# Lucaskabela/UNAST

Measured on AMD Instinct MI355X. Metric: mel-frames/sec/node (train step, gen+disc) at B=32,T_mel=800; 1/2/4/8-GPU scaling, higher is better.
Workload: dtype bf16x3

## Files before the change

### include/unast_hip.h

```cpp
#ifndef UNAST_HIP_H
#define UNAST_HIP_H
#include <stdint.h>
#ifdef __cplusplus
extern "C" {
#endif

typedef struct ihipStream_t* hipStream_t;

const char* unast_last_error(void);
int unast_version(void);
const char* unast_arch(void);

int unast_gemm(int a_mode, int b_mode, int nsplit,
               const float* A, int lda, const float* B, int ldb, float* C, int ldc,
               int M, int N, int K, int kb_valid,
               int conv_T, int conv_ca, int conv_cb, int conv_shift,
               const float* bias, const float* R, int ldr, const float* G, int ldg, float gate_scale,
               float alpha, int beta, int act,
               float drop_p, unsigned int seed, unsigned int stream_id,
               int splitk, float* splitk_ws, int64_t splitk_ws_floats, float* rowsum_a, int tile_wn, int b_presplit,
               int out_split, double* colstats, hipStream_t stream);

int unast_attn_fwd(int nsplit, const float* Q, int ldq, const float* K, int ldk, const float* V, int ldv, float* O, int ldo,
                   float* LSE, const int* lens_k, int B, int H, int Tq, int Tk, int head_dim, int causal, float scale,
// ... 83 lines not shown
                        double* ws, float* loss, hipStream_t stream);
int unast_text_loss_bwd(const float* logits, int ldl, const int64_t* gold, int rows, int V, float eos_weight, const double* ws,
                        const float* gscale, float* dlogits, hipStream_t stream);
int unast_text_head_loss(const float* X, int ldx, const float* W, const float* bias, const int64_t* gold, int rows, int K, int V,
                         float eos_weight, float gscale, float* logits, float* dlogits, int ldl, double* ws, float* loss, hipStream_t stream);
int unast_speech_head_loss(const float* X, int ldx, const float* W, const float* bias, const float* gold, const int* lens, int B, int T, int K, int M,
                           float eos_weight, float gscale, float* head, float* d_head, int ldh, double* ws, hipStream_t stream);
int unast_speech_post_loss(const float* gold, const float* post, const int* lens, int B, int T, int M, float gscale, float* d_post, double* ws,
                           float* loss, hipStream_t stream);
int unast_disc_targets(const int64_t* perm, int n, int B, int flip, float smoothing, float* out, hipStream_t stream);
int unast_randperm(int64_t* out, int n, unsigned int seed, unsigned int stream_id, hipStream_t stream);
int unast_bce_logits(const float* logits, int ldx, const float* targets, int n, const float* gscale, float* loss, float* dlogits,
                     int ldd, hipStream_t stream);

int unast_lstm_fwd(const float* xproj, const float* whh, const float* b_ih, const float* b_hh, const int* lens, float* y, float* gates,
                   float* cs, float* hprev, float* hfinal, int Bd, int T, int ndir, int hidden, int64_t whh_dir_stride,
                   int64_t bias_dir_stride, hipStream_t stream);
int unast_lstm_bwd(const float* dy, const float* dhfinal, const float* whh, const float* gates, const float* cs, const int* lens,
                   float* dgates, int Bd, int T, int ndir, int hidden, int64_t whh_dir_stride, hipStream_t stream);
int unast_leaky_dropout(const float* x, const float* dy, float* out, int rows, int D, float slope, float drop_p, unsigned int seed,
                        unsigned int stream_id, hipStream_t stream);

int unast_conv_fwd(int nsplit, const float* X, int ldx, const float* Wp, float* Y, int ldy, int B, int T, int Cin, int Cout,
                   int taps, int pad_left, const float* bias, int act, const float* R, int ldr, hipStream_t stream);
int unast_maxpool_prev(const float* in, int ld_in, float* out, int ld_out, int B, int T, int C, hipStream_t stream);
int unast_highway_combine(const float* ht, int ld_ht, const float* x, int ld_x, float* out, int ld_out, int rows, int C, hipStream_t stream);
int unast_gru_fwd(const float* xproj, const float* whh, const float* b_hn, float* y, int B, int T, int hidden, hipStream_t stream);

int unast_set_rng_epoch(const unsigned int* counter);

typedef struct {
    const float* A; int lda;
    const float* B; int ldb;
    float* C; int ldc;
    float* rowsum_a;
    int M, N, K;
} unast_wgrad_item;
int unast_wgrad_group(int nsplit, int count, const unast_wgrad_item* items, float* ws, int64_t ws_floats, int target_blocks,
                      hipStream_t stream);
int64_t unast_wgrad_group_ws_floats(int count, const unast_wgrad_item* items, int target_blocks);

int unast_sumsq(const float* g, int64_t n, double* out, hipStream_t stream);
int unast_adamw(float* p, float* g, float* m, float* v, int64_t n, const double* sumsq, float max_norm, float lr,
                float beta1, float beta2, float eps, float weight_decay, int step, float* split_out, int decoupled,
                const float* dev_hyper, int zero_grad, hipStream_t stream);
int unast_split_f32(const float* src, float* dst, int64_t n, hipStream_t stream);
int unast_transpose_split(const float* src_base, float* dst_base, const int* tiles_dev, int ntiles, hipStream_t stream);

int unast_panel_gemm(const float* A, int lda, const void* w_planes, int64_t plane_bytes, float* C, int ldc, int M, int N, int K,
                     const float* bias, const float* R, int ldr, const float* G, int ldg, float gate_scale, int act,
                     float drop_p, unsigned int seed, unsigned int stream_id, int out_split,
                     const float* ln_gamma, const float* ln_beta, float* Y, int ldy, float* mean, float* rstd, float eps,
                     void* gate_bits, int rows_per_wg, hipStream_t stream);
int unast_retile_weights(const float* src_base, void* dst_base, const void* descs_dev, int ndesc, hipStream_t stream);
int unast_panel_gemm_lnbwd(const float* A, int lda, const void* w_planes, int64_t plane_bytes, int M, int K, const float* R, int ldr,
                           const float* z, int ldz, const float* mean, const float* rstd, const float* gamma,
                           float* dz, int lddz, float* dz_drop, int lddrop, float* part, int64_t part_floats,
                           float drop_p, unsigned int seed, unsigned int stream_id, hipStream_t stream);
int64_t unast_panel_gemm_lnbwd_ws_floats(int M);
int unast_layernorm_partials_finalize(const float* part, int nblk, int C, float* dgamma, float* dbeta, hipStream_t stream);
int unast_set_words(unsigned int* dst, const unsigned int* host_words, int n, hipStream_t stream);

int64_t unast_graph_plan_create(void* graph, int nstreams);
int unast_graph_plan_info(int64_t plan, int* out4);
int unast_graph_plan_replay(int64_t plan, hipStream_t origin);
int unast_graph_plan_destroy(int64_t plan);
int unast_graph_plan_allreduces(int64_t plan);
int unast_graph_plan_set_comm(int64_t plan, int64_t comm);
int unast_graph_plan_allreduce_counts(int64_t plan, long long* out, int n);
int unast_capture_reset(void);
int unast_capture_note(hipStream_t stream);
int unast_capture_get_deps(hipStream_t stream, void** out, int cap);
int unast_capture_prune(hipStream_t stream, hipStream_t origin, void** keep, int nkeep);
int unast_graph_plan_streams(int64_t plan);

int unast_comm_unique_id(void* out128);
int64_t unast_comm_init(const void* unique_id128, int rank, int world);
int unast_allreduce(int64_t comm, float* buf, int64_t count, hipStream_t stream);
int unast_allreduce_marker(float* buf, int64_t count, hipStream_t stream);
int unast_comm_destroy(int64_t comm);

#ifdef __cplusplus
}
#endif
#endif
```

### unast_amd/config.py

```python
import os

NSPLIT = 1 if os.environ.get("UNAST_PREC", "bf16x3").lower() in ("bf16", "1") else 3


def set_precision(name):
    global NSPLIT
    NSPLIT = {"bf16": 1, "bf16x3": 3}[name]


def precision_name():
    return "bf16" if NSPLIT == 1 else "bf16x3"


def snapshot():
    return tuple(sorted((k, v) for k, v in globals().items() if k.isupper()))


SIDE_STREAMS = os.environ.get("UNAST_SIDE_STREAMS", "1") != "0"

DECODE_GRAPH = os.environ.get("UNAST_DECODE_GRAPH", "1") != "0"

WGRAD_STREAM_MIN_TOKENS = int(os.environ.get("UNAST_WGRAD_MIN_TOKENS", "8192"))

DETERMINISTIC_SUMS = os.environ.get("UNAST_DETERMINISTIC_SUMS", "0") == "1"

CAPTURE_PRUNE = os.environ.get("UNAST_CAPTURE_PRUNE", "1") != "0"

WGRAD_GROUP = os.environ.get("UNAST_WGRAD_GROUP", "1") != "0"

ATTN_FUSED_BWD = os.environ.get("UNAST_ATTN_FUSED_BWD", "1") != "0"
ATTN_BWD_TERMS = int(os.environ.get("UNAST_ATTN_BWD_TERMS", "3"))

DGRAD_TRANSPOSED = os.environ.get("UNAST_DGRAD_T", "0") == "1"

PANEL_MIN_ROWS = int(os.environ.get("UNAST_PANEL_MIN_ROWS", "16384"))
PANEL_ROWS = int(os.environ.get("UNAST_PANEL_ROWS", "1128"))

NATIVE_COMM = os.environ.get("UNAST_NATIVE_COMM", "1") != "0"

ENC_SKIP_PAD_GRADS = os.environ.get("UNAST_ENC_SKIP_PAD_GRADS", "0") == "1"

STREAM_JITTER = int(os.environ.get("UNAST_STREAM_JITTER", "0"))
STREAM_JITTER_SEED = int(os.environ.get("UNAST_STREAM_JITTER_SEED", "0"))

DEBUG_WORKSPACES = os.environ.get("UNAST_DEBUG_WORKSPACES", "0") == "1"

JOINT_GEN = os.environ.get("UNAST_JOINT_GEN", "1") != "0"
```

### unast_amd/csrc/panel.hip

```cpp
#include "common.h"
#include <algorithm>
#include "../../include/unast_hip.h"
#include <type_traits>

static unsigned long long* g_panel_stamps = nullptr;
#define PSUB 1024

struct PanelParams {
    const float* A; int lda;
    const unsigned char* W; size_t plane_bytes;
    float* C; int ldc;
    int M, N, K, ncg;
    const float* bias; const float* R; int ldr;
    const float* G; int ldg; float gate_scale;
    int act; uint32_t drop_thresh; float drop_scale; uint32_t seed, stream;
    int out_split;
    const float* gamma; const float* beta; float* Y; int ldy; float* mean; float* rstd; float eps;
    const float* Z; int ldz; float* part;
    unsigned long long* gate_bits;
    unsigned long long* stamps;
};

__device__ __forceinline__ void panel_wait_vm(int n) {
#define PW(k) asm volatile("s_waitcnt vmcnt(" #k ")" ::: "memory")
    if (n < 8) {
        if (n < 4) { if (n < 2) PW(0); else PW(2); }
        else       { if (n < 6) PW(4); else PW(6); }
    } else if (n < 16) {
        if (n < 12) { if (n < 10) PW(8); else PW(10); }
        else        { if (n < 14) PW(12); else PW(14); }
    } else {
        if (n < 20) PW(16); else PW(20);
    }
#undef PW
}

#ifdef PANEL_STAMPS
__device__ __forceinline__ unsigned long long panel_stamp() {
    unsigned long long t;
    asm volatile("s_memtime %0\n\ts_waitcnt lgkmcnt(0)" : "=s"(t) :: "memory");
    return t;
}
#define STAMP(var) const unsigned long long var = panel_stamp()
#define STAMP_ADD(slot, a, b) stamp_sum[slot] += (b) - (a)
#else
#define STAMP(var)
#define STAMP_ADD(slot, a, b)
#endif

template <int KSTEPS, int RT, int LN, int NW>
__global__ __launch_bounds__(64 * NW, NW / 4) void panel_kernel(const PanelParams p) {
    constexpr int NT = 64 * NW, ROWS = (NW / 2) * 16 * RT;
    constexpr int NSUB = 8 * KSTEPS;
    constexpr int GROUP = NSUB * PSUB;
    constexpr int DMAX = (NSUB + NW - 1) / NW;
    constexpr int RING = 2 * GROUP;
    constexpr bool A_DMA = (KSTEPS == 8);
    static_assert(!A_DMA || RING >= ROWS * 1024, "the A image borrows the ring");
    __shared__ __attribute__((aligned(16))) unsigned char smem[(RING > ROWS * 1024 || !A_DMA ? RING : ROWS * 1024) + 4096 + 1024];

    const int t = threadIdx.x, lane = t & 63, l15 = lane & 15, g = lane >> 4;
    const int wave = __builtin_amdgcn_readfirstlane(t >> 6);
    __builtin_assume(wave >= 0 && wave < NW);
    const int rg = wave >> 1, ch = wave & 1;
    const int m_wg = blockIdx.x * ROWS;
    const int m_wave = m_wg + rg * (16 * RT);
#ifdef PANEL_STAMPS
    unsigned long long stamp_sum[8] = {0, 0, 0, 0, 0, 0, 0, 0};
    const unsigned long long t_begin = panel_stamp();
#endif
    const uint32_t rbase = p.drop_thresh ? rng_stream_base(p.seed, p.stream) : 0u;

    const __amdgpu_buffer_rsrc_t w_rsrc = __builtin_amdgcn_make_buffer_rsrc(const_cast<unsigned char*>(p.W), 0, 0x7FFFFFF0, 0x00020000);
    const int lane16 = lane * 16;
    auto issue_group = [&](int cg) {
#pragma unroll
        for (int q = 0; q < DMAX; ++q) {
            const int j = wave + NW * q;
            if (j >= NSUB) break;
            const int pl = j / (4 * KSTEPS), rem = j - pl * (4 * KSTEPS);
            const uint32_t soff = (uint32_t)pl * (uint32_t)p.plane_bytes + (uint32_t)(4 * cg * KSTEPS + rem) * PSUB;
            __builtin_amdgcn_raw_ptr_buffer_load_lds(w_rsrc, (__attribute__((address_space(3))) void*)(smem + (cg & 1) * GROUP + j * PSUB), 16, lane16, (int)soff, 0, 0);
        }
    };

    float* const sbias = reinterpret_cast<float*>(smem + RING);
    float* const sred = sbias + 1024;
    const uint32_t sbias_lds = (uint32_t)(uintptr_t)(__attribute__((address_space(3))) void*)sbias;
    const bool bias_lds = p.bias && p.N <= 1024;
    if (bias_lds) {
        for (int i = t; i < 64 * p.ncg; i += NT) sbias[i] = (i < p.N) ? p.bias[i] : 0.f;
    }

    bf16x8_t ah[RT][KSTEPS], al[RT][KSTEPS];
    if constexpr (A_DMA) {
        const __amdgpu_buffer_rsrc_t a_rsrc = __builtin_amdgcn_make_buffer_rsrc(const_cast<float*>(p.A), 0, 0x7FFFFFF0, 0x00020000);
#pragma unroll
        for (int q = 0; q < ROWS / NW; ++q) {
            const int r = wave * (ROWS / NW) + q;
            const int row = min(m_wg + r, p.M - 1);
            __builtin_amdgcn_raw_ptr_buffer_load_lds(a_rsrc, (__attribute__((address_space(3))) void*)(smem + r * 1024), 16, (lane ^ (r & 15)) << 4,
                                                     (int)((uint32_t)row * (uint32_t)p.lda * 4u), 0, 0);
        }
        asm volatile("s_waitcnt vmcnt(0)" ::: "memory");
        __syncthreads();
#pragma unroll
        for (int rt = 0; rt < RT; ++rt) {
            const unsigned char* rowp = smem + (rg * (16 * RT) + 16 * rt + l15) * 1024;
#pragma unroll
            for (int ks = 0; ks < KSTEPS; ++ks) {
                const int c0 = 8 * ks + 2 * g;
                const float4 a = *reinterpret_cast<const float4*>(rowp + ((c0 ^ l15) << 4));
                const float4 c = *reinterpret_cast<const float4*>(rowp + (((c0 + 1) ^ l15) << 4));
                u32x2 h0, l0, h1, l1;
                split4<3>(a, h0, l0);
                split4<3>(c, h1, l1);
                ah[rt][ks] = __builtin_bit_cast(bf16x8_t, (u32x4){h0[0], h0[1], h1[0], h1[1]});
                al[rt][ks] = __builtin_bit_cast(bf16x8_t, (u32x4){l0[0], l0[1], l1[0], l1[1]});
            }
        }
        __syncthreads();
    } else {
#pragma unroll
        for (int rt = 0; rt < RT; ++rt) {
            const int row = min(m_wave + 16 * rt + l15, p.M - 1);
            const float* ar = p.A + (size_t)row * p.lda;
#pragma unroll
            for (int ks = 0; ks < KSTEPS; ++ks) {
                const int k = 32 * ks + 8 * g;
                const int k0 = min(k, p.K - 4), k1 = min(k + 4, p.K - 4);
                float4 a = *reinterpret_cast<const float4*>(ar + k0);
                float4 c = *reinterpret_cast<const float4*>(ar + k1);
                if (k >= p.K) a = make_float4(0.f, 0.f, 0.f, 0.f);
                if (k + 4 >= p.K) c = make_float4(0.f, 0.f, 0.f, 0.f);
                u32x2 h0, l0, h1, l1;
                split4<3>(a, h0, l0);
                split4<3>(c, h1, l1);
                ah[rt][ks] = __builtin_bit_cast(bf16x8_t, (u32x4){h0[0], h0[1], h1[0], h1[1]});
                al[rt][ks] = __builtin_bit_cast(bf16x8_t, (u32x4){l0[0], l0[1], l1[0], l1[1]});
            }
        }
        __syncthreads();
    }
    issue_group(0);
#ifdef PANEL_STAMPS
    { const unsigned long long tp = panel_stamp(); stamp_sum[5] = tp - t_begin; }
#endif

    const bool vec_c = (p.ldc & 3) == 0;
    const bool vec_r = p.R && (p.ldr & 3) == 0 && ((((uintptr_t)p.R) & 15) == 0);
    const bool vec_g = p.G && (p.ldg & 3) == 0 && ((((uintptr_t)p.G) & 15) == 0);
    const int lane_off = (g * 16 + l15) * 16;

    auto epilogue = [&](int cg, f32x4 (&ac)[RT][2]) {
#pragma unroll
        for (int rt = 0; rt < RT; ++rt) {
            const int m = m_wave + 16 * rt + l15;
            if (m >= p.M) continue;
            uint32_t rkey = 0;
            if (p.drop_thresh) rkey = pcg_hash((uint32_t)m + rbase);
#pragma unroll
            for (int c2 = 0; c2 < 2; ++c2) {
                const int n = 64 * cg + 32 * ch + 16 * c2 + 4 * g;
                if (n >= p.N) continue;
                float v[4] = {ac[rt][c2][0], ac[rt][c2][1], ac[rt][c2][2], ac[rt][c2][3]};
                float bv[4] = {0.f, 0.f, 0.f, 0.f}, gv[4] = {1.f, 1.f, 1.f, 1.f}, rv[4] = {0.f, 0.f, 0.f, 0.f};
                const bool full = n + 3 < p.N;
                if (p.bias) {
#pragma unroll
                    for (int r = 0; r < 4; ++r) bv[r] = (n + r < p.N) ? p.bias[n + r] : 0.f;
                }
                if (p.G) {
                    if (full && vec_g) { const float4 t4 = *reinterpret_cast<const float4*>(p.G + (size_t)m * p.ldg + n); gv[0] = t4.x; gv[1] = t4.y; gv[2] = t4.z; gv[3] = t4.w; }
                    else { for (int r = 0; r < 4; ++r) if (n + r < p.N) gv[r] = p.G[(size_t)m * p.ldg + n + r]; }
                }
                if (p.R) {
                    if (full && vec_r) { const float4 t4 = *reinterpret_cast<const float4*>(p.R + (size_t)m * p.ldr + n); rv[0] = t4.x; rv[1] = t4.y; rv[2] = t4.z; rv[3] = t4.w; }
                    else { for (int r = 0; r < 4; ++r) if (n + r < p.N) rv[r] = p.R[(size_t)m * p.ldr + n + r]; }
                }
#pragma unroll
                for (int r = 0; r < 4; ++r) {
                    float x = v[r] + bv[r];
                    if (p.act == 1) x = fmaxf(x, 0.f);
                    if (p.drop_thresh) x = rng_keep(rkey, (uint32_t)(n + r), p.drop_thresh) ? x * p.drop_scale : 0.f;
                    if (p.G) x = (gv[r] > 0.f) ? x * p.gate_scale : 0.f;
                    v[r] = x + rv[r];
                }
                float* cp = p.C + (size_t)m * p.ldc + n;
                if (full && vec_c) {
                    const float4 o = make_float4(v[0], v[1], v[2], v[3]);
                    if (p.out_split) *reinterpret_cast<uint4*>(cp) = split_chunk(o);
                    else *reinterpret_cast<float4*>(cp) = o;
                } else {
                    for (int r = 0; r < 4; ++r) if (n + r < p.N) cp[r] = v[r];
                }
            }
        }
    };
    const __amdgpu_buffer_rsrc_t c_rsrc = __builtin_amdgcn_make_buffer_rsrc(p.C, 0, (int)min((size_t)0x7FFFFFF0, ((size_t)(p.M - 1) * p.ldc + p.N) * 4), 0x00020000);
    uint32_t c_voff[RT], c_rkey[RT];
#pragma unroll
    for (int rt = 0; rt < RT; ++rt) {
        const int m = m_wave + 16 * rt + l15;
        c_voff[rt] = ((uint32_t)m * (uint32_t)p.ldc + (uint32_t)(32 * ch + 4 * g)) * 4u;
        c_rkey[rt] = pcg_hash((uint32_t)m + rbase);
    }
    const int ntile_n = (p.N + 15) >> 4, ntile_m = (p.M + 15) >> 4;
    const __amdgpu_buffer_rsrc_t g_rsrc = __builtin_amdgcn_make_buffer_rsrc(p.gate_bits, 0, ((p.M + 127) >> 7) * 8 * ntile_n * 32, 0x00020000);
    auto epilogue_fast = [&](int cg, f32x4 (&ac)[RT][2], auto act_t, auto drop_t, auto split_t, auto wbits_t, auto rgate_t) {
        constexpr bool ACT = decltype(act_t)::value, DROP = decltype(drop_t)::value, SPLIT = decltype(split_t)::value;
        constexpr bool WBITS = decltype(wbits_t)::value, RGATE = decltype(rgate_t)::value;
        f32x4 b4[2] = {(f32x4){0.f, 0.f, 0.f, 0.f}, (f32x4){0.f, 0.f, 0.f, 0.f}};
        if (bias_lds) {
            const uint32_t ba = sbias_lds + 4u * (uint32_t)(64 * cg + 32 * ch + 4 * g);
            asm volatile("ds_read_b128 %0, %2\n\tds_read_b128 %1, %2 offset:64\n\ts_waitcnt lgkmcnt(0)" : "=&v"(b4[0]), "=&v"(b4[1]) : "v"(ba) : "memory");
        }
        const int soff = cg * 256;
#pragma unroll
        for (int rt = 0; rt < RT; ++rt) {
#pragma unroll
            for (int c2 = 0; c2 < 2; ++c2) {
                float v[4] = {ac[rt][c2][0] + b4[c2][0], ac[rt][c2][1] + b4[c2][1], ac[rt][c2][2] + b4[c2][2], ac[rt][c2][3] + b4[c2][3]};
                if (ACT) {
#pragma unroll
                    for (int r = 0; r < 4; ++r) asm("v_max_f32 %0, 0, %1" : "=v"(v[r]) : "v"(v[r]));
                }
                if (DROP) {
                    const uint32_t n = (uint32_t)(64 * cg + 32 * ch + 16 * c2 + 4 * g);
                    const uint32_t h01 = rng_pair(c_rkey[rt], n), h23 = rng_pair(c_rkey[rt], n + 2u);
                    v[0] = rng_keep_lo(h01, p.drop_thresh) ? v[0] * p.drop_scale : 0.f;
                    v[1] = rng_keep_hi(h01, p.drop_thresh) ? v[1] * p.drop_scale : 0.f;
                    v[2] = rng_keep_lo(h23, p.drop_thresh) ? v[2] * p.drop_scale : 0.f;
                    v[3] = rng_keep_hi(h23, p.drop_thresh) ? v[3] * p.drop_scale : 0.f;
                }
                if (WBITS || RGATE) {
                    const int tile_m = RGATE ? min((m_wave >> 4) + rt, ntile_m - 1) : (m_wave >> 4) + rt;
                    const int widx = ((tile_m * ntile_n) + 4 * cg + 2 * ch + c2) * 4;
                    if (WBITS) {
                        const unsigned long long b0 = __ballot(v[0] > 0.f), b1 = __ballot(v[1] > 0.f), b2 = __ballot(v[2] > 0.f), b3 = __ballot(v[3] > 0.f);
                        const unsigned long long mine = lane == 0 ? b0 : lane == 1 ? b1 : lane == 2 ? b2 : b3;
                        if (lane < 4) __builtin_amdgcn_raw_buffer_store_b64((u32x2){(uint32_t)mine, (uint32_t)(mine >> 32)}, g_rsrc, (widx + lane) * 8, 0, 0);
                    } else {
                        const __attribute__((address_space(4))) unsigned long long* wp = (const __attribute__((address_space(4))) unsigned long long*)(uintptr_t)p.gate_bits + widx;
#pragma unroll
                        for (int r = 0; r < 4; ++r) v[r] = ((wp[r] >> lane) & 1ull) ? v[r] * p.gate_scale : 0.f;
                    }
                }
                u32x4 o;
                if (SPLIT) {
                    const uint4 sc = split_chunk(make_float4(v[0], v[1], v[2], v[3]));
                    o = (u32x4){sc.x, sc.y, sc.z, sc.w};
                } else {
                    o = (u32x4){__float_as_uint(v[0]), __float_as_uint(v[1]), __float_as_uint(v[2]), __float_as_uint(v[3])};
                }
                __builtin_amdgcn_raw_buffer_store_b128(o, c_rsrc, (int)(c_voff[rt] + (uint32_t)soff) + 64 * c2, 0, 0);
            }
        }
    };
    const int s_fast = 2 * RT;
    int st_prev = 0, st_now = 0;
    const bool fast_ok = vec_c && !p.R && !p.G && (bias_lds || !p.bias);
    const int epi_kind = !fast_ok ? 0 : p.gate_bits ? (p.act == 1 ? (p.out_split ? 0 : p.drop_thresh ? 5 : 7) : (!p.drop_thresh && !p.out_split && !p.bias ? 6 : 0))
                       : p.drop_thresh ? (p.act == 1 && !p.out_split ? 1 : 0) : p.out_split ? (p.act == 1 ? 0 : 2) : (p.act == 1 ? 3 : 4);
    const int s_epi = s_fast + (epi_kind == 5 || epi_kind == 7 ? 2 * RT : 0);
    auto run_epilogue = [&](int cg, f32x4 (&ac)[RT][2]) {
        STAMP(te0);
        using T = std::true_type; using F = std::false_type;
#ifdef PKO_PLAIN_EPILOGUE
        if (64 * cg + 64 <= p.N) { epilogue_fast(cg, ac, F{}, F{}, F{}, F{}, F{}); st_now += s_fast; return; }
#endif
#ifdef PKO_NO_EPILOGUE
        if (64 * cg + 64 <= p.N) { asm volatile("" :: "v"(ac[0][0]), "v"(ac[0][1])); return; }
#endif
        if (epi_kind == 0 || 64 * cg + 64 > p.N) {
            epilogue(cg, ac);
        } else {
            __builtin_amdgcn_s_setprio(1);
            if (epi_kind == 1) epilogue_fast(cg, ac, T{}, T{}, F{}, F{}, F{});
            else if (epi_kind == 2) epilogue_fast(cg, ac, F{}, F{}, T{}, F{}, F{});
            else if (epi_kind == 3) epilogue_fast(cg, ac, T{}, F{}, F{}, F{}, F{});
            else if (epi_kind == 5) epilogue_fast(cg, ac, T{}, T{}, F{}, T{}, F{});
            else if (epi_kind == 6) epilogue_fast(cg, ac, F{}, F{}, F{}, F{}, T{});
            else if (epi_kind == 7) epilogue_fast(cg, ac, T{}, F{}, F{}, T{}, F{});
            else epilogue_fast(cg, ac, F{}, F{}, F{}, F{}, F{});
            __builtin_amdgcn_s_setprio(0);
            st_now += s_epi;
        }
        STAMP(te1);
        STAMP_ADD(3, te0, te1);
    };

    auto group_sync = [&](int cg) {
        STAMP(ta);
        panel_wait_vm(st_prev);
        STAMP(tb);
        __builtin_amdgcn_s_barrier();
        STAMP(tc);
        if (cg + 1 < p.ncg) issue_group(cg + 1);
        STAMP(td);
        STAMP_ADD(0, ta, tb); STAMP_ADD(1, tb, tc); STAMP_ADD(2, tc, td);
    };
    auto group_mma = [&](int cg, auto k0_t, auto k1_t, f32x4 (&ac)[RT][2]) {
        constexpr int K0 = decltype(k0_t)::value, K1 = decltype(k1_t)::value;
        if constexpr (K0 < K1) {
            const unsigned char* base = smem + (cg & 1) * GROUP + lane_off + (2 * ch) * KSTEPS * PSUB;
            bf16x8_t bf[2][2][2];
            auto load_b = [&](int buf, int ks) {
#pragma unroll
                for (int c2 = 0; c2 < 2; ++c2) {
                    bf[buf][c2][0] = *reinterpret_cast<const bf16x8_t*>(base + ((0 * 4 + c2) * KSTEPS + ks) * PSUB);
                    bf[buf][c2][1] = *reinterpret_cast<const bf16x8_t*>(base + ((1 * 4 + c2) * KSTEPS + ks) * PSUB);
                }
            };
            STAMP(tm0);
            load_b(K0 & 1, K0);
#ifdef PKO_NO_LDS_READS
            load_b((K0 + 1) & 1, K0);
#endif
#pragma unroll
            for (int ks = K0; ks < K1; ++ks) {
#ifndef PKO_NO_LDS_READS
                if (ks + 1 < K1) load_b((ks + 1) & 1, ks + 1);
#endif
#pragma unroll
                for (int c2 = 0; c2 < 2; ++c2) {
                    const bf16x8_t bh = bf[ks & 1][c2][0], bl = bf[ks & 1][c2][1];
#pragma unroll
                    for (int rt = 0; rt < RT; ++rt) {
#ifndef PKO_ONE_MFMA
                        ac[rt][c2] = mfma16(bl, ah[rt][ks], ac[rt][c2]);
                        ac[rt][c2] = mfma16(bh, al[rt][ks], ac[rt][c2]);
#endif
                        ac[rt][c2] = mfma16(bh, ah[rt][ks], ac[rt][c2]);
                    }
                }
            }
#ifdef PANEL_STAMPS
            asm volatile("" :: "v"(ac[0][0]), "v"(ac[0][1]));
#endif
            STAMP(tm1);
            STAMP_ADD(4, tm0, tm1);
        }
    };
    auto end_iteration = [&]() { st_prev = st_now; st_now = 0; };
    constexpr int KH = (KSTEPS + 1) / 2;
    using I0 = std::integral_constant<int, 0>; using IH = std::integral_constant<int, KH>; using IK = std::integral_constant<int, KSTEPS>;
    auto zero = [&](f32x4 (&ac)[RT][2]) {
#pragma unroll
        for (int rt = 0; rt < RT; ++rt) { ac[rt][0] = (f32x4){0.f, 0.f, 0.f, 0.f}; ac[rt][1] = ac[rt][0]; }
    };

// ... 31 lines not shown
                        s1[rt] += x;
                    }
                }
            s1[rt] += __shfl_xor(s1[rt], 16, 64);
            s1[rt] += __shfl_xor(s1[rt], 32, 64);
        }
        if (g == 0) {
#pragma unroll
            for (int rt = 0; rt < RT; ++rt) sred[((rg * 2 + ch) * RT + rt) * 16 + l15] = s1[rt];
        }
        __syncthreads();
        float mu[RT], s2[RT];
#pragma unroll
        for (int rt = 0; rt < RT; ++rt) {
            mu[rt] = (s1[rt] + sred[((rg * 2 + (ch ^ 1)) * RT + rt) * 16 + l15]) * (1.f / 256.f);
            s2[rt] = 0.f;
#pragma unroll
            for (int cg = 0; cg < 4; ++cg)
#pragma unroll
                for (int c2 = 0; c2 < 2; ++c2)
#pragma unroll
                    for (int r = 0; r < 4; ++r) { const float d = zv[rt][cg][c2][r] - mu[rt]; s2[rt] += d * d; }
            s2[rt] += __shfl_xor(s2[rt], 16, 64);
            s2[rt] += __shfl_xor(s2[rt], 32, 64);
        }
        __syncthreads();
        if (g == 0) {
#pragma unroll
            for (int rt = 0; rt < RT; ++rt) sred[((rg * 2 + ch) * RT + rt) * 16 + l15] = s2[rt];
        }
        __syncthreads();
#pragma unroll
        for (int rt = 0; rt < RT; ++rt) {
            const int m = m_wave + 16 * rt + l15;
            const float rs = rsqrtf((s2[rt] + sred[((rg * 2 + (ch ^ 1)) * RT + rt) * 16 + l15]) * (1.f / 256.f) + p.eps);
            if (m >= p.M) continue;
            if (g == 0 && ch == 0) { p.mean[m] = mu[rt]; p.rstd[m] = rs; }
#pragma unroll
            for (int cg = 0; cg < 4; ++cg)
#pragma unroll
                for (int c2 = 0; c2 < 2; ++c2) {
                    const int n = 64 * cg + 32 * ch + 16 * c2 + 4 * g;
                    const float4 g4 = *reinterpret_cast<const float4*>(p.gamma + n), b4 = *reinterpret_cast<const float4*>(p.beta + n);
                    const float* z = zv[rt][cg][c2];
                    *reinterpret_cast<float4*>(p.C + (size_t)m * p.ldc + n) = make_float4(z[0], z[1], z[2], z[3]);
                    *reinterpret_cast<float4*>(p.Y + (size_t)m * p.ldy + n) =
                        make_float4((z[0] - mu[rt]) * rs * g4.x + b4.x, (z[1] - mu[rt]) * rs * g4.y + b4.y, (z[2] - mu[rt]) * rs * g4.z + b4.z, (z[3] - mu[rt]) * rs * g4.w + b4.w);
                }
        }
    } else {
        const bool late = ((wave >> 2) & 1) != 0;
        f32x4 acc[RT][2], pend[RT][2];
        zero(acc);
        for (int cg = 0; cg < p.ncg; ++cg) {
            group_sync(cg);
            if (!late && cg > 0) run_epilogue(cg - 1, pend);
            group_mma(cg, I0{}, IH{}, acc);
            if (late && cg > 0) run_epilogue(cg - 1, pend);
            group_mma(cg, IH{}, IK{}, acc);
            end_iteration();
#pragma unroll
            for (int rt = 0; rt < RT; ++rt) { pend[rt][0] = acc[rt][0]; pend[rt][1] = acc[rt][1]; }
            zero(acc);
        }
        run_epilogue(p.ncg - 1, pend);
    }
    asm volatile("s_waitcnt vmcnt(0)" ::: "memory");
#ifdef PANEL_STAMPS
    if (p.stamps && lane == 0) {
        stamp_sum[6] = panel_stamp() - t_begin;
        for (int k = 0; k < 8; ++k) p.stamps[((size_t)blockIdx.x * 8 + wave) * 8 + k] = stamp_sum[k];
    }
#endif
}

typedef __attribute__((ext_vector_type(16))) float f32x16_t;
__global__ __launch_bounds__(512, 1) void panel32_kernel(const PanelParams p) {
    constexpr int KSTEPS = 8, NW = 8, NT = 64 * NW, ROWS = 128;
    constexpr int NSUB = 8 * KSTEPS, GROUP = NSUB * PSUB, DMAX = NSUB / NW, RING = 2 * GROUP;
    static_assert(RING >= ROWS * 1024, "the A image borrows the ring");
    __shared__ __attribute__((aligned(16))) unsigned char smem[RING + 4096 + 1024];
    const int t = threadIdx.x, lane = t & 63, l31 = lane & 31, kh = lane >> 5;
    const int wave = __builtin_amdgcn_readfirstlane(t >> 6);
    __builtin_assume(wave >= 0 && wave < NW);
    const int rg = wave >> 1, ch = wave & 1;
    const int m_wg = blockIdx.x * ROWS, m_wave = m_wg + 32 * rg;
    const uint32_t rbase = p.drop_thresh ? rng_stream_base(p.seed, p.stream) : 0u;
    const __amdgpu_buffer_rsrc_t w_rsrc = __builtin_amdgcn_make_buffer_rsrc(const_cast<unsigned char*>(p.W), 0, 0x7FFFFFF0, 0x00020000);
    const int lane16 = lane * 16;
    auto issue_group = [&](int cg) {
#pragma unroll
        for (int q = 0; q < DMAX; ++q) {
            const int j = wave + NW * q;
            const int pl = j / (4 * KSTEPS), rem = j - pl * (4 * KSTEPS);
            const uint32_t soff = (uint32_t)pl * (uint32_t)p.plane_bytes + (uint32_t)(4 * cg * KSTEPS + rem) * PSUB;
            __builtin_amdgcn_raw_ptr_buffer_load_lds(w_rsrc, (__attribute__((address_space(3))) void*)(smem + (cg & 1) * GROUP + j * PSUB), 16, lane16, (int)soff, 0, 0);
        }
    };
    float* const sbias = reinterpret_cast<float*>(smem + RING);
    const uint32_t sbias_lds = (uint32_t)(uintptr_t)(__attribute__((address_space(3))) void*)sbias;
    const bool bias_lds = p.bias != nullptr;
    if (bias_lds) for (int i = t; i < 64 * p.ncg; i += NT) sbias[i] = (i < p.N) ? p.bias[i] : 0.f;

    bf16x8_t ah[16], al[16];
    {
        const __amdgpu_buffer_rsrc_t a_rsrc = __builtin_amdgcn_make_buffer_rsrc(const_cast<float*>(p.A), 0, 0x7FFFFFF0, 0x00020000);
#pragma unroll
        for (int q = 0; q < ROWS / NW; ++q) {
            const int r = wave * (ROWS / NW) + q;
            const int row = min(m_wg + r, p.M - 1);
            __builtin_amdgcn_raw_ptr_buffer_load_lds(a_rsrc, (__attribute__((address_space(3))) void*)(smem + r * 1024), 16, (lane ^ (r & 15)) << 4,
                                                     (int)((uint32_t)row * (uint32_t)p.lda * 4u), 0, 0);
        }
        asm volatile("s_waitcnt vmcnt(0)" ::: "memory");
        __syncthreads();
        const unsigned char* rowp = smem + (32 * rg + l31) * 1024;
        const int sw = l31 & 15;
#pragma unroll
        for (int ks = 0; ks < 16; ++ks) {
// ... 409 lines not shown
            }
            s1[rt] += __shfl_xor(s1[rt], 16, 64);
            s1[rt] += __shfl_xor(s1[rt], 32, 64);
        }
        if (g == 0) {
#pragma unroll
            for (int rt = 0; rt < 2; ++rt) sred[ch * 128 + 32 * rg + 16 * rt + l15] = s1[rt];
        }
        __syncthreads();
#pragma unroll
        for (int rt = 0; rt < 2; ++rt) {
            const int r0 = 32 * rg + 16 * rt + l15;
            mu[rt] = ((sred[r0] + sred[128 + r0]) + (sred[256 + r0] + sred[384 + r0])) * (1.f / 256.f);
            s2[rt] = 0.f;
#pragma unroll
            for (int ct = 0; ct < 4; ++ct)
#pragma unroll
                for (int r = 0; r < 4; ++r) { const float d = acc[rt][ct][r] - mu[rt]; s2[rt] += d * d; }
            s2[rt] += __shfl_xor(s2[rt], 16, 64);
            s2[rt] += __shfl_xor(s2[rt], 32, 64);
        }
        __syncthreads();
        if (g == 0) {
#pragma unroll
            for (int rt = 0; rt < 2; ++rt) sred[ch * 128 + 32 * rg + 16 * rt + l15] = s2[rt];
        }
        __syncthreads();
#pragma unroll
        for (int rt = 0; rt < 2; ++rt) {
            const int r0 = 32 * rg + 16 * rt + l15, m = m_wg + r0;
            const float rs = rsqrtf(((sred[r0] + sred[128 + r0]) + (sred[256 + r0] + sred[384 + r0])) * (1.f / 256.f) + p.eps);
            if (m >= p.M) continue;
            if (g == 0 && ch == 0) { p.mean[m] = mu[rt]; p.rstd[m] = rs; }
#pragma unroll
            for (int ct = 0; ct < 4; ++ct) {
                const int n = 64 * ch + 16 * ct + 4 * g;
                const float4 g4 = *reinterpret_cast<const float4*>(p.gamma + n), b4 = *reinterpret_cast<const float4*>(p.beta + n);
                const f32x4 z = acc[rt][ct];
                *reinterpret_cast<float4*>(p.C + (size_t)m * p.ldc + n) = make_float4(z[0], z[1], z[2], z[3]);
                *reinterpret_cast<float4*>(p.Y + (size_t)m * p.ldy + n) =
                    make_float4((z[0] - mu[rt]) * rs * g4.x + b4.x, (z[1] - mu[rt]) * rs * g4.y + b4.y, (z[2] - mu[rt]) * rs * g4.z + b4.z, (z[3] - mu[rt]) * rs * g4.w + b4.w);
            }
        }
    }
#ifdef PANEL_STAMPS
    if (p.stamps && lane == 0) {
        const unsigned long long t_end = panel_stamp();
        stamp_sum[6] = t_end - t_begin; stamp_sum[7] = t_end - t_loop;
        for (int k = 0; k < 8; ++k) p.stamps[((size_t)(blockIdx.x * gridDim.y + blockIdx.y) * 16 + wave) * 8 + k] = stamp_sum[k];
    }
#endif
}

template <int KSTEPS>
static void panel_launch(const PanelParams& p, int rows, int ln, hipStream_t s) {
    const int r = rows == 1128 ? 128 : rows;
    dim3 grid((p.M + r - 1) / r);
    if (rows == 1128) {
        if (ln) hipLaunchKernelGGL((panel_kernel<KSTEPS, 1, 1, 16>), grid, dim3(1024), 0, s, p);
        else    hipLaunchKernelGGL((panel_kernel<KSTEPS, 1, 0, 16>), grid, dim3(1024), 0, s, p);
    } else if (ln) {
        if (rows == 128) hipLaunchKernelGGL((panel_kernel<KSTEPS, 2, 1, 8>), grid, dim3(512), 0, s, p);
        else             hipLaunchKernelGGL((panel_kernel<KSTEPS, 1, 1, 8>), grid, dim3(512), 0, s, p);
    } else {
        if (rows == 128) hipLaunchKernelGGL((panel_kernel<KSTEPS, 2, 0, 8>), grid, dim3(512), 0, s, p);
        else             hipLaunchKernelGGL((panel_kernel<KSTEPS, 1, 0, 8>), grid, dim3(512), 0, s, p);
    }
}

extern "C" int64_t unast_panel_gemm_lnbwd_ws_floats(int M) { return (int64_t)((M + 127) / 128) * 2 * 256; }

extern "C" int unast_panel_gemm_lnbwd(const float* A, int lda, const void* w_planes, int64_t plane_bytes, int M, int K, const float* R, int ldr,
                                      const float* z, int ldz, const float* mean, const float* rstd, const float* gamma,
                                      float* dz, int lddz, float* dz_drop, int lddrop, float* part, int64_t part_floats,
                                      float drop_p, unsigned int seed, unsigned int stream_id, hipStream_t stream) {
    UNAST_REQUIRE(A && w_planes && z && mean && rstd && gamma && dz && M > 0, "unast_panel_gemm_lnbwd: null pointer");
    UNAST_REQUIRE(K > 256 && (K & 63) == 0 && (lda & 3) == 0 && (lddz & 3) == 0 && (ldz & 3) == 0 && (!R || (ldr & 3) == 0) && (!dz_drop || (lddrop & 3) == 0) &&
                  ((((uintptr_t)A) | ((uintptr_t)dz) | ((uintptr_t)w_planes) | ((uintptr_t)z) | ((uintptr_t)R) | ((uintptr_t)dz_drop) | ((uintptr_t)gamma)) & 15) == 0,
                  "unast_panel_gemm_lnbwd: needs K > 256, K %% 64 == 0, 16-byte row strides and aligned operands (K=%d)", K);
    UNAST_REQUIRE(!part || part_floats >= unast_panel_gemm_lnbwd_ws_floats(M), "unast_panel_gemm_lnbwd: partials buffer too small");
    UNAST_REQUIRE(dz_drop || drop_p <= 0.f, "unast_panel_gemm_lnbwd: dropout needs the second output");
    {
        const size_t ld_max = (size_t)std::max(std::max(lda, lddz), std::max(std::max(R ? ldr : 0, ldz), dz_drop ? lddrop : 0));
        UNAST_REQUIRE(((size_t)M + 127) / 128 * 128 * ld_max * 4 < (size_t)0x7FFFFFF0u, "unast_panel_gemm_lnbwd: operand exceeds the 2 GiB a buffer descriptor addresses");
    }
    PanelParams q = {};
    q.stamps = nullptr;
    q.A = A; q.lda = lda; q.W = (const unsigned char*)w_planes; q.plane_bytes = (size_t)plane_bytes; q.C = dz; q.ldc = lddz; q.M = M; q.N = 256; q.K = K; q.ncg = 4;
    q.R = R; q.ldr = ldr; q.Z = z; q.ldz = ldz; q.mean = const_cast<float*>(mean); q.rstd = const_cast<float*>(rstd); q.gamma = gamma;
    q.Y = dz_drop; q.ldy = lddrop; q.part = part;
    q.drop_thresh = dz_drop ? drop_threshold(drop_p) : 0u; q.drop_scale = drop_p > 0.f ? 1.f / (1.f - drop_p) : 1.f; q.seed = seed; q.stream = stream_id;
    hipLaunchKernelGGL((kpanel_kernel<2>), dim3((M + 127) / 128, 1), dim3(1024), 0, stream, q);
    return unast_check_launch("unast_panel_gemm_lnbwd");
}

extern "C" int unast_panel_debug_stamps(void* dev_buf) { g_panel_stamps = (unsigned long long*)dev_buf; return 0; }

extern "C" int unast_panel_gemm(const float* A, int lda, const void* w_planes, int64_t plane_bytes, float* C, int ldc, int M, int N, int K,
                                const float* bias, const float* R, int ldr, const float* G, int ldg, float gate_scale, int act,
                                float drop_p, unsigned int seed, unsigned int stream_id, int out_split,
                                const float* ln_gamma, const float* ln_beta, float* Y, int ldy, float* mean, float* rstd, float eps,
                                void* gate_bits, int rows_per_wg, hipStream_t stream) {
    UNAST_REQUIRE(A && w_planes && C && M > 0 && N > 0 && K >= 4, "unast_panel_gemm: bad arguments");
    {
        const size_t ld_max = (size_t)std::max(std::max(lda, ldc), std::max(R ? ldr : 0, Y ? ldy : 0));
        UNAST_REQUIRE(((size_t)M + 127) / 128 * 128 * ld_max * 4 < (size_t)0x7FFFFFF0u, "unast_panel_gemm: operand of %d rows x %zu floats exceeds the 2 GiB a buffer descriptor addresses (use unast_gemm)", M, ld_max);
    }
    if (K > 256) {
        UNAST_REQUIRE((K & 63) == 0 && (N & 255) == 0 && (lda & 3) == 0 && (ldc & 3) == 0 && ((((uintptr_t)A) | ((uintptr_t)C) | ((uintptr_t)w_planes)) & 15) == 0,
                      "unast_panel_gemm: K > 256 needs K %% 64 == 0, N %% 256 == 0, 16-byte row strides and aligned operands (N=%d K=%d)", N, K);
        UNAST_REQUIRE(!G && !act && !out_split && !gate_bits, "unast_panel_gemm: K > 256 serves the plain, residual and LayerNorm epilogues only");
        UNAST_REQUIRE(!R || ((ldr & 3) == 0 && (((uintptr_t)R) & 15) == 0), "unast_panel_gemm: residual operand must be 16-byte addressable");
// ... 55 lines not shown
```

### unast_amd/ops.py

```python
import os as _os

import torch

from . import config
from ._lib import lib, check

OP_KC, OP_KC_CONV, OP_RC, OP_RC_CONV_DGRAD, OP_RC_CONV_WGRAD = 0, 1, 2, 3, 4


def _p(t):
    return None if t is None else t.data_ptr()


_raw_stream = getattr(torch._C, "_cuda_getCurrentRawStream", None)


def _stream():
    if _raw_stream is not None:
        return _raw_stream(torch.cuda.current_device())
    return torch.cuda.current_stream().cuda_stream


_F32 = torch.float32
_LN_WS = {}
# ... 291 lines not shown
    n = len(chunk)
    arr = (_WgradItem * n)()
    operands = []
    for j, (dy2d, x2d, dW, db) in enumerate(chunk):
        a = arr[j]
        a.A, a.lda, a.B, a.ldb, a.C, a.ldc = dy2d.data_ptr(), dy2d.stride(0), x2d.data_ptr(), x2d.stride(0), dW.data_ptr(), dW.stride(0)
        a.rowsum_a = db.data_ptr() if db is not None else None
        a.M, a.N, a.K = dy2d.shape[1], x2d.shape[1], dy2d.shape[0]
        operands += [dy2d, x2d]
    ptr = _ct.addressof(arr)
    ws_n = lib().unast_wgrad_group_ws_floats(n, ptr, WGRAD_GROUP_TARGET)
    if ws_n <= 0:
        raise RuntimeError("unast_wgrad_group_ws_floats failed")

    shapes = tuple((int(a.M), int(a.N), int(a.K), int(a.rowsum_a is not None)) for a in arr)

    def launch():
        import sys
        sys.modules[__name__].wgrad_group(shapes, n, ptr, ws_n, chunk[0][0].device)
    if offload:
        w = WGRAD_SIDE()
        from . import engine
        engine.wait(w, torch.cuda.current_stream())
        for t in operands:
            t.record_stream(w)
        with torch.cuda.stream(w):
            launch()
    else:
        launch()


def wgrad_group(shapes, n, items_ptr, ws_n, device):
    ws = torch.empty(ws_n, dtype=torch.float32, device=device)
    check(lib().unast_wgrad_group(config.NSPLIT, n, items_ptr, _p(ws), ws_n, WGRAD_GROUP_TARGET, _stream()), "unast_wgrad_group")


def linear_wgrad(dy2d, x2d, dW, db=None):
    if _BATCH is not None and _groupable(dy2d, x2d, dW, db):
        _BATCH.append((dy2d, x2d, dW, db))
        return dW
    return _linear_wgrad_now(dy2d, x2d, dW, db)


_PANEL_TRACE = _os.environ.get("UNAST_PANEL_TRACE", "0") == "1"


def retile_weights(src_flat, dst_bytes, descs_dev, ndesc):
    check(lib().unast_retile_weights(_p(src_flat), _p(dst_bytes), _p(descs_dev), ndesc, _stream()), "unast_retile_weights")


PANEL_LAUNCHES = [0, 0]


def panel_gemm(A, wplanes, C, N, bias=None, R=None, G=None, gate_scale=1.0, act=0, drop_p=0.0, seed=0, stream_id=0, out_split=False,
               ln=None, rows_per_wg=0, K=None, gate_bits=None):
    M = A.shape[0]
    K = A.shape[1] if K is None else K
    g = b = Y = mean = rstd = None
    eps, ldy = 0.0, 0
    if ln is not None:
        g, b, Y, mean, rstd, eps = ln
        ldy = Y.stride(0)
    PANEL_LAUNCHES[0 if K <= 256 else 1] += 1
    if _PANEL_TRACE:
        print("panel_gemm M=%d N=%d K=%d lda=%d ldc=%d bias=%s R=%s G=%s act=%d drop=%.2f split=%d ln=%s bits=%s rows=%d" % (
            M, N, K, A.stride(0), C.stride(0), bias is not None, R is not None, G is not None, act, drop_p, out_split, ln is not None,
            None if gate_bits is None else gate_bits.numel(), rows_per_wg), flush=True)
    check(lib().unast_panel_gemm(_p(A), A.stride(0), wplanes[0], wplanes[1], _p(C), C.stride(0), M, N, K, _p(bias), _p(R),
                                 R.stride(0) if R is not None else 0, _p(G), G.stride(0) if G is not None else 0, gate_scale, act,
                                 drop_p, seed & 0xFFFFFFFF, stream_id, int(out_split), _p(g), _p(b), _p(Y), ldy, _p(mean), _p(rstd), eps,
                                 _p(gate_bits), rows_per_wg, _stream()), "unast_panel_gemm")
    if _PANEL_TRACE:
        torch.cuda.synchronize()
    return C


def conv_fwd(x3d, Wp, bias, out, pad_left, colstats=None):
    B, T, Cin = x3d.shape
    Cout = Wp.shape[0]
    gemm(OP_KC_CONV, OP_KC, x3d, x3d.stride(1), Wp, 5 * Cin, out, out.stride(1), B * T, Cout, 5 * Cin,
         conv=(T, Cin, 0, pad_left), bias=bias, colstats=colstats)
    return out


def conv_dgrad(dy3d, Wp, dx, pad_left, beta=0):
    B, T, Cout = dy3d.shape
    Cin = Wp.shape[2]
    gemm(OP_KC_CONV, OP_RC_CONV_DGRAD, dy3d, dy3d.stride(1), Wp, 4, dx, dx.stride(1), B * T, Cin, 5 * Cout,
         conv=(T, Cout, Cout, 4 - pad_left), beta=beta)
    return dx


def conv_wgrad(dy3d, x3d, dWp, pad_left, db=None):
    B, T, Cout = dy3d.shape
    Cin = x3d.shape[2]
    sk = _splitk_for(Cout, 5 * Cin, B * T)
    if db is not None and deterministic_sums() and dy3d.is_contiguous():
        def both():
            gemm(OP_RC, OP_RC_CONV_WGRAD, dy3d, dy3d.stride(1), x3d, x3d.stride(1), dWp, 5 * Cin, Cout, 5 * Cin, B * T,
                 conv=(T, 0, Cin, pad_left), beta=1, splitk=sk)
            colsum(dy3d.view(B * T, Cout), db)
        _on_wgrad_stream(both, B * T, dWp.data_ptr(), dy3d, x3d)
        return dWp
    _on_wgrad_stream(lambda: gemm(OP_RC, OP_RC_CONV_WGRAD, dy3d, dy3d.stride(1), x3d, x3d.stride(1), dWp, 5 * Cin, Cout, 5 * Cin, B * T,
                                  conv=(T, 0, Cin, pad_left), beta=1, splitk=sk, rowsum_a=db), B * T, dWp.data_ptr(), dy3d, x3d)
    return dWp


# ... 412 lines not shown
```

Measured before the change: 929,200.

## Balance panel GEMM work across CUs with contiguous panel/column-group item ranges

Adds a balanced variant of the panel GEMM kernel. The grid is capped at the CU count, and each workgroup processes a contiguous range of (row-panel, column-group) items, so the partial last wave of panels no longer leaves CUs idle. A host-side cost model decides per shape whether balancing beats the plain launch, using empirical per-panel and per-group costs and a margin. The price is extra A-panel reloads at segment boundaries, an additional barrier, and the model's heuristic constants. It applies only to non-LayerNorm launches with K<=256 and is on by default.

```diff
diff --git a/include/unast_hip.h b/include/unast_hip.h
--- a/include/unast_hip.h
+++ b/include/unast_hip.h
@@ -159,6 +159,9 @@
                      float drop_p, unsigned int seed, unsigned int stream_id, int out_split,
                      const float* ln_gamma, const float* ln_beta, float* Y, int ldy, float* mean, float* rstd, float eps,
                      void* gate_bits, int rows_per_wg, hipStream_t stream);
+int unast_panel_schedule(int M, int N, int K, int n_cu, int* first_item, int cap);
+int unast_panel_balance(int mode);
+int unast_panel_balance_cus(int n_cu);
 int unast_retile_weights(const float* src_base, void* dst_base, const void* descs_dev, int ndesc, hipStream_t stream);
 int unast_panel_gemm_lnbwd(const float* A, int lda, const void* w_planes, int64_t plane_bytes, int M, int K, const float* R, int ldr,
                            const float* z, int ldz, const float* mean, const float* rstd, const float* gamma,
diff --git a/unast_amd/config.py b/unast_amd/config.py
--- a/unast_amd/config.py
+++ b/unast_amd/config.py
@@ -35,6 +35,7 @@
 
 PANEL_MIN_ROWS = int(os.environ.get("UNAST_PANEL_MIN_ROWS", "16384"))
 PANEL_ROWS = int(os.environ.get("UNAST_PANEL_ROWS", "1128"))
+PANEL_BALANCE = os.environ.get("UNAST_PANEL_BALANCE", "1") != "0"
 
 NATIVE_COMM = os.environ.get("UNAST_NATIVE_COMM", "1") != "0"
 
diff --git a/unast_amd/csrc/panel.hip b/unast_amd/csrc/panel.hip
--- a/unast_amd/csrc/panel.hip
+++ b/unast_amd/csrc/panel.hip
@@ -48,8 +48,9 @@
 #define STAMP_ADD(slot, a, b)
 #endif
 
-template <int KSTEPS, int RT, int LN, int NW>
+template <int KSTEPS, int RT, int LN, int NW, int BAL = 0>
 __global__ __launch_bounds__(64 * NW, NW / 4) void panel_kernel(const PanelParams p) {
+    static_assert(!BAL || !LN, "the LayerNorm epilogue needs whole rows in one workgroup");
     constexpr int NT = 64 * NW, ROWS = (NW / 2) * 16 * RT;
     constexpr int NSUB = 8 * KSTEPS;
     constexpr int GROUP = NSUB * PSUB;
@@ -63,8 +64,17 @@
     const int wave = __builtin_amdgcn_readfirstlane(t >> 6);
     __builtin_assume(wave >= 0 && wave < NW);
     const int rg = wave >> 1, ch = wave & 1;
-    const int m_wg = blockIdx.x * ROWS;
-    const int m_wave = m_wg + rg * (16 * RT);
+    int m_wg = blockIdx.x * ROWS;
+    int m_wave = m_wg + rg * (16 * RT);
+    int c0 = 0, c1 = p.ncg;
+    uint32_t item = 0, item_end = 0;
+    if constexpr (BAL) {
+        const uint32_t T = (uint32_t)((p.M + ROWS - 1) / ROWS) * (uint32_t)p.ncg;
+        item = blockIdx.x * T / gridDim.x;
+        item_end = (blockIdx.x + 1) * T / gridDim.x;
+        if (item >= item_end) return;
+    }
+    bool first_segment = true;
 #ifdef PANEL_STAMPS
     unsigned long long stamp_sum[8] = {0, 0, 0, 0, 0, 0, 0, 0};
     const unsigned long long t_begin = panel_stamp();
@@ -92,6 +102,17 @@
         for (int i = t; i < 64 * p.ncg; i += NT) sbias[i] = (i < p.N) ? p.bias[i] : 0.f;
     }
 
+    do {
+    if constexpr (BAL) {
+        const uint32_t pn = item / (uint32_t)p.ncg;
+        c0 = (int)(item - pn * (uint32_t)p.ncg);
+        c1 = min(p.ncg, c0 + (int)(item_end - item));
+        item += (uint32_t)(c1 - c0);
+        m_wg = (int)pn * ROWS;
+        m_wave = m_wg + rg * (16 * RT);
+        if (!first_segment) __syncthreads();
+        first_segment = false;
+    }
     bf16x8_t ah[RT][KSTEPS], al[RT][KSTEPS];
     if constexpr (A_DMA) {
         const __amdgpu_buffer_rsrc_t a_rsrc = __builtin_amdgcn_make_buffer_rsrc(const_cast<float*>(p.A), 0, 0x7FFFFFF0, 0x00020000);
@@ -104,14 +125,16 @@
         }
         asm volatile("s_waitcnt vmcnt(0)" ::: "memory");
         __syncthreads();
+        int sw = l15;
+        if constexpr (BAL) asm volatile("" : "+v"(sw));
 #pragma unroll
         for (int rt = 0; rt < RT; ++rt) {
-            const unsigned char* rowp = smem + (rg * (16 * RT) + 16 * rt + l15) * 1024;
+            const unsigned char* rowp = smem + (rg * (16 * RT) + 16 * rt + sw) * 1024;
 #pragma unroll
             for (int ks = 0; ks < KSTEPS; ++ks) {
                 const int c0 = 8 * ks + 2 * g;
-                const float4 a = *reinterpret_cast<const float4*>(rowp + ((c0 ^ l15) << 4));
-                const float4 c = *reinterpret_cast<const float4*>(rowp + (((c0 + 1) ^ l15) << 4));
+                const float4 a = *reinterpret_cast<const float4*>(rowp + ((c0 ^ sw) << 4));
+                const float4 c = *reinterpret_cast<const float4*>(rowp + (((c0 + 1) ^ sw) << 4));
                 u32x2 h0, l0, h1, l1;
                 split4<3>(a, h0, l0);
                 split4<3>(c, h1, l1);
@@ -142,7 +165,7 @@
         }
         __syncthreads();
     }
-    issue_group(0);
+    issue_group(c0);
 #ifdef PANEL_STAMPS
     { const unsigned long long tp = panel_stamp(); stamp_sum[5] = tp - t_begin; }
 #endif
@@ -210,9 +233,11 @@
     auto epilogue_fast = [&](int cg, f32x4 (&ac)[RT][2], auto act_t, auto drop_t, auto split_t, auto wbits_t, auto rgate_t) {
         constexpr bool ACT = decltype(act_t)::value, DROP = decltype(drop_t)::value, SPLIT = decltype(split_t)::value;
         constexpr bool WBITS = decltype(wbits_t)::value, RGATE = decltype(rgate_t)::value;
+        int lane_e = lane;
+        if constexpr (BAL) asm volatile("" : "+v"(lane_e));
         f32x4 b4[2] = {(f32x4){0.f, 0.f, 0.f, 0.f}, (f32x4){0.f, 0.f, 0.f, 0.f}};
         if (bias_lds) {
-            const uint32_t ba = sbias_lds + 4u * (uint32_t)(64 * cg + 32 * ch + 4 * g);
+            const uint32_t ba = sbias_lds + 4u * (uint32_t)(64 * cg + 32 * ch + 4 * (BAL ? lane_e >> 4 : g));
             asm volatile("ds_read_b128 %0, %2\n\tds_read_b128 %1, %2 offset:64\n\ts_waitcnt lgkmcnt(0)" : "=&v"(b4[0]), "=&v"(b4[1]) : "v"(ba) : "memory");
         }
         const int soff = cg * 256;
@@ -239,7 +264,7 @@
                     if (WBITS) {
                         const unsigned long long b0 = __ballot(v[0] > 0.f), b1 = __ballot(v[1] > 0.f), b2 = __ballot(v[2] > 0.f), b3 = __ballot(v[3] > 0.f);
                         const unsigned long long mine = lane == 0 ? b0 : lane == 1 ? b1 : lane == 2 ? b2 : b3;
-                        if (lane < 4) __builtin_amdgcn_raw_buffer_store_b64((u32x2){(uint32_t)mine, (uint32_t)(mine >> 32)}, g_rsrc, (widx + lane) * 8, 0, 0);
+                        if (lane < 4) __builtin_amdgcn_raw_buffer_store_b64((u32x2){(uint32_t)mine, (uint32_t)(mine >> 32)}, g_rsrc, (widx + lane_e) * 8, 0, 0);
                     } else {
                         const __attribute__((address_space(4))) unsigned long long* wp = (const __attribute__((address_space(4))) unsigned long long*)(uintptr_t)p.gate_bits + widx;
 #pragma unroll
@@ -296,7 +321,7 @@
         STAMP(tb);
         __builtin_amdgcn_s_barrier();
         STAMP(tc);
-        if (cg + 1 < p.ncg) issue_group(cg + 1);
+        if (cg + 1 < c1) issue_group(cg + 1);
         STAMP(td);
         STAMP_ADD(0, ta, tb); STAMP_ADD(1, tb, tc); STAMP_ADD(2, tc, td);
     };
@@ -434,19 +459,20 @@
         const bool late = ((wave >> 2) & 1) != 0;
         f32x4 acc[RT][2], pend[RT][2];
         zero(acc);
-        for (int cg = 0; cg < p.ncg; ++cg) {
+        for (int cg = c0; cg < c1; ++cg) {
             group_sync(cg);
-            if (!late && cg > 0) run_epilogue(cg - 1, pend);
+            if (!late && cg > c0) run_epilogue(cg - 1, pend);
             group_mma(cg, I0{}, IH{}, acc);
-            if (late && cg > 0) run_epilogue(cg - 1, pend);
+            if (late && cg > c0) run_epilogue(cg - 1, pend);
             group_mma(cg, IH{}, IK{}, acc);
             end_iteration();
 #pragma unroll
             for (int rt = 0; rt < RT; ++rt) { pend[rt][0] = acc[rt][0]; pend[rt][1] = acc[rt][1]; }
             zero(acc);
         }
-        run_epilogue(p.ncg - 1, pend);
-    }
+        run_epilogue(c1 - 1, pend);
+    }
+    } while (BAL && item < item_end);
     asm volatile("s_waitcnt vmcnt(0)" ::: "memory");
 #ifdef PANEL_STAMPS
     if (p.stamps && lane == 0) {
@@ -962,12 +988,86 @@
 #endif
 }
 
+struct PanelCost { float P, g; };
+static PanelCost panel_cost(int ksteps) {
+    switch (ksteps) {
+        case 8: return {5.7f, 2.9f};
+        case 4: return {5.4f, 1.8f};
+        case 3: return {3.9f, 1.6f};
+        default: return {0.f, 0.f};
+    }
+}
+#define PANEL_BAL_MARGIN 0.06f
+
+static int g_panel_balance = 1;
+static int g_panel_cus = 0;
+
+static int panel_device_cus() {
+    static const int n = [] {
+        int dev = 0;
+        hipDeviceProp_t pr;
+        if (hipGetDevice(&dev) != hipSuccess || hipGetDeviceProperties(&pr, dev) != hipSuccess) return 0;
+        return (int)pr.multiProcessorCount;
+    }();
+    return n;
+}
+
+static int panel_balance_wgs(int M, int N, int K, int n_cu, int mode) {
+#ifdef PANEL_STAMPS
+    return 0;
+#endif
+    if (mode == 0 || M <= 0 || N <= 0 || K < 4 || K > 256 || n_cu <= 0) return 0;
+    const long long panels = ((long long)M + 127) / 128, ncg = ((long long)N + 63) / 64, T = panels * ncg;
+    const long long G = std::min<long long>(n_cu, panels);
+    if (T * (G + 1) >= (1ll << 31)) return 0;
+    if (mode == 2) return (int)G;
+    const long long rounds = (panels + n_cu - 1) / n_cu;
+    if (rounds < 2) return 0;
+    long long maxseg = 1;
+    for (long long i = 0; i < G; ++i) {
+        const long long a = i * T / G, b = (i + 1) * T / G;
+        maxseg = std::max(maxseg, (b - 1) / ncg - a / ncg + 1);
+    }
+    const PanelCost c = panel_cost((K + 31) / 32);
+    if (c.P <= 0.f) return 0;
+    const float plain = (float)rounds * (c.P + (float)ncg * c.g);
+    const float bal = (float)maxseg * c.P + (float)((T + G - 1) / G) * c.g;
+    return bal < plain * (1.f - PANEL_BAL_MARGIN) ? (int)G : 0;
+}
+
+extern "C" int unast_panel_schedule(int M, int N, int K, int n_cu, int* first_item, int cap) {
+    const int G = panel_balance_wgs(M, N, K, n_cu, g_panel_balance);
+    if (G > 0 && first_item) {
+        const long long T = (((long long)M + 127) / 128) * (((long long)N + 63) / 64);
+        for (int i = 0; i <= G && i < cap; ++i) first_item[i] = (int)((long long)i * T / G);
+    }
+    return G;
+}
+
+extern "C" int unast_panel_balance(int mode) {
+    const int old = g_panel_balance;
+    if (mode >= 0 && mode <= 2) g_panel_balance = mode;
+    return old;
+}
+
+extern "C" int unast_panel_balance_cus(int n_cu) {
+    const int old = g_panel_cus;
+    if (n_cu >= 0) g_panel_cus = n_cu;
+    return old;
+}
+
 template <int KSTEPS>
 static void panel_launch(const PanelParams& p, int rows, int ln, hipStream_t s) {
     const int r = rows == 1128 ? 128 : rows;
     dim3 grid((p.M + r - 1) / r);
     if (rows == 1128) {
-        if (ln) hipLaunchKernelGGL((panel_kernel<KSTEPS, 1, 1, 16>), grid, dim3(1024), 0, s, p);
+        static thread_local int memo_key[8][5], memo_wgs[8];
+        const int n_cu = g_panel_cus > 0 ? g_panel_cus : panel_device_cus();
+        const int key[5] = {p.M, p.N, p.K, n_cu, g_panel_balance + 1}, slot = (p.M / 128 + p.N / 64 + p.K / 32) & 7;
+        if (!std::equal(key, key + 5, memo_key[slot])) { memo_wgs[slot] = panel_balance_wgs(p.M, p.N, p.K, n_cu, g_panel_balance); std::copy(key, key + 5, memo_key[slot]); }
+        const int bal_wgs = ln ? 0 : memo_wgs[slot];
+        if (bal_wgs) hipLaunchKernelGGL((panel_kernel<KSTEPS, 1, 0, 16, 1>), dim3(bal_wgs), dim3(1024), 0, s, p);
+        else if (ln) hipLaunchKernelGGL((panel_kernel<KSTEPS, 1, 1, 16>), grid, dim3(1024), 0, s, p);
         else    hipLaunchKernelGGL((panel_kernel<KSTEPS, 1, 0, 16>), grid, dim3(1024), 0, s, p);
     } else if (ln) {
         if (rows == 128) hipLaunchKernelGGL((panel_kernel<KSTEPS, 2, 1, 8>), grid, dim3(512), 0, s, p);
diff --git a/unast_amd/ops.py b/unast_amd/ops.py
--- a/unast_amd/ops.py
+++ b/unast_amd/ops.py
@@ -367,8 +367,15 @@
 PANEL_LAUNCHES = [0, 0]
 
 
+_PANEL_BALANCE_MODE = [None]
+
+
 def panel_gemm(A, wplanes, C, N, bias=None, R=None, G=None, gate_scale=1.0, act=0, drop_p=0.0, seed=0, stream_id=0, out_split=False,
-               ln=None, rows_per_wg=0, K=None, gate_bits=None):
+               ln=None, rows_per_wg=0, K=None, gate_bits=None, balance=None):
+    mode = (1 if config.PANEL_BALANCE else 0) if balance is None else int(balance)
+    if mode != _PANEL_BALANCE_MODE[0]:
+        lib().unast_panel_balance(mode)
+        _PANEL_BALANCE_MODE[0] = mode
     M = A.shape[0]
     K = A.shape[1] if K is None else K
     g = b = Y = mean = rstd = None
```

Result: no change. 935,000 (median of 6 runs) (+0.6%).
